# Sanoojan/REFace

Hardware: AMD Instinct MI355X
Metric: 512x512 50-step DDIM images/sec (higher is better)
Workload: dtype bf16; 1 GPU; BASELINE configs[1]: 512x512, 50 DDIM steps, CFG scale 3.5, batch 8 per GPU, bf16 UNet + fp32 VAE decode (bf16x3 MFMA operands), seeded random-init REFace weights; id=c1:512x512:S50:B8:bf16, batch_per_gpu=8, global_batch=8, ddim_steps=50, latent=64, parallelism=dp1 (pairs sharded, no collective in the step loop)

## Files before the change

### reface_amd/csrc/common.h

```cpp
#pragma once
#include <hip/hip_runtime.h>
#include <stdint.h>
#include <stdio.h>
#include <stdlib.h>
#include <string.h>

#include "../../include/reface_hip.h"

typedef __attribute__((ext_vector_type(8))) __bf16 bf16x8_t;
typedef __attribute__((ext_vector_type(16))) float f32x16_t;
typedef __attribute__((ext_vector_type(4))) float f32x4_t;
typedef __attribute__((ext_vector_type(4))) uint32_t u32x4_t;
typedef __attribute__((ext_vector_type(2))) uint32_t u32x2_t;

typedef uint16_t bf16_t;
typedef _Float16 f16_t;
typedef __attribute__((ext_vector_type(8))) _Float16 f16x8_t;
typedef uint8_t fp8_t;

namespace rf {

void set_error(const char* fmt, ...);


// ... 17 lines not shown
#define RF_RAISE_LDS(kernel, bytes, name)                                                                                                   \
    do {                                                                                                                                    \
        static unsigned long long done_ = 0ull;                                                                                             \
        int dev_ = 0;                                                                                                                       \
        (void)hipGetDevice(&dev_);                                                                                                          \
        const unsigned long long bit_ = 1ull << (dev_ & 63);                                                                                \
        if (!(done_ & bit_)) {                                                                                                              \
            const hipError_t e_ = hipFuncSetAttribute((const void*)(kernel), hipFuncAttributeMaxDynamicSharedMemorySize, (bytes));          \
            if (e_ != hipSuccess) {                                                                                                         \
                rf::set_error("%s: cannot raise the dynamic LDS limit to %d bytes on device %d: %s", name, (int)(bytes), dev_, hipGetErrorString(e_)); \
                return 2;                                                                                                                   \
            }                                                                                                                               \
            done_ |= bit_;                                                                                                                  \
        }                                                                                                                                   \
    } while (0)

__device__ __forceinline__ float as_f32(uint32_t x) { return __builtin_bit_cast(float, x); }
__device__ __forceinline__ uint32_t as_u32(float x) { return __builtin_bit_cast(uint32_t, x); }

typedef __attribute__((ext_vector_type(2))) __bf16 bf16x2_t;
__device__ __forceinline__ uint32_t pack_bf2(float lo, float hi) {
    const bf16x2_t v = {(__bf16)lo, (__bf16)hi};
    return __builtin_bit_cast(uint32_t, v);
}
__device__ __forceinline__ bf16_t f2bf(float f) { return __builtin_bit_cast(bf16_t, (__bf16)f); }
__device__ __forceinline__ float bf2f(bf16_t h) { return as_f32(((uint32_t)h) << 16); }

typedef __attribute__((ext_vector_type(2))) _Float16 f16x2_t;
__device__ __forceinline__ uint32_t pack_h2(float lo, float hi) {
    const f16x2_t v = {(_Float16)lo, (_Float16)hi};
    return __builtin_bit_cast(uint32_t, v);
}
template <typename T> __device__ __forceinline__ uint32_t pack2(float lo, float hi);
template <> __device__ __forceinline__ uint32_t pack2<bf16_t>(float lo, float hi) { return pack_bf2(lo, hi); }
template <> __device__ __forceinline__ uint32_t pack2<f16_t>(float lo, float hi) { return pack_h2(lo, hi); }
template <typename T> __device__ __forceinline__ float lo16(uint32_t w);
template <typename T> __device__ __forceinline__ float hi16(uint32_t w);
template <> __device__ __forceinline__ float lo16<bf16_t>(uint32_t w) { return as_f32(w << 16); }
template <> __device__ __forceinline__ float hi16<bf16_t>(uint32_t w) { return as_f32(w & 0xffff0000u); }
template <> __device__ __forceinline__ float lo16<f16_t>(uint32_t w) { return (float)__builtin_bit_cast(f16x2_t, w)[0]; }
template <> __device__ __forceinline__ float hi16<f16_t>(uint32_t w) { return (float)__builtin_bit_cast(f16x2_t, w)[1]; }
template <typename T> __device__ __forceinline__ float round16(float v);
template <> __device__ __forceinline__ float round16<bf16_t>(float v) { return bf2f(f2bf(v)); }
template <> __device__ __forceinline__ float round16<f16_t>(float v) { return (float)(_Float16)v; }
template <typename T> __device__ __forceinline__ constexpr uint16_t one16();
template <> __device__ __forceinline__ constexpr uint16_t one16<bf16_t>() { return 0x3f80; }
template <> __device__ __forceinline__ constexpr uint16_t one16<f16_t>() { return 0x3c00; }

__device__ __forceinline__ void split4_bf16(const float* f, u32x2_t& hi, u32x2_t& lo) {
    hi[0] = pack_bf2(f[0], f[1]);
    hi[1] = pack_bf2(f[2], f[3]);
    const float r0 = f[0] - as_f32(hi[0] << 16), r1 = f[1] - as_f32(hi[0] & 0xffff0000u);
    const float r2 = f[2] - as_f32(hi[1] << 16), r3 = f[3] - as_f32(hi[1] & 0xffff0000u);
    lo[0] = pack_bf2(r0, r1);
    lo[1] = pack_bf2(r2, r3);
}

__device__ __forceinline__ float quad_max(float v) {
    v = fmaxf(v, as_f32((uint32_t)__builtin_amdgcn_mov_dpp((int)as_u32(v), 0xB1, 0xF, 0xF, true)));
    v = fmaxf(v, as_f32((uint32_t)__builtin_amdgcn_mov_dpp((int)as_u32(v), 0x4E, 0xF, 0xF, true)));
    return v;
}
__device__ __forceinline__ int e8m0_for_amax(float amax) {
    const uint32_t b = as_u32(amax);
    int c = (int)((b >> 23) & 0xffu) - 8 + ((b & 0x7fffffu) > 0x600000u ? 1 : 0);
    return c < 0 ? 0 : (c > 253 ? 253 : c);
}
__device__ __forceinline__ u32x2_t quant8_fp8(const float* f, int code) {
    const float inv = as_f32((uint32_t)(254 - code) << 23);
    int lo = 0, hi = 0;
    lo = __builtin_amdgcn_cvt_pk_fp8_f32(f[0] * inv, f[1] * inv, lo, false);
    lo = __builtin_amdgcn_cvt_pk_fp8_f32(f[2] * inv, f[3] * inv, lo, true);
    hi = __builtin_amdgcn_cvt_pk_fp8_f32(f[4] * inv, f[5] * inv, hi, false);
    hi = __builtin_amdgcn_cvt_pk_fp8_f32(f[6] * inv, f[7] * inv, hi, true);
    return u32x2_t{(uint32_t)lo, (uint32_t)hi};
}
__device__ __forceinline__ void quant_block8(const float* f, fp8_t* qdst, fp8_t* sdst, bool quad_leader) {
    float m = 0.f;
#pragma unroll
    for (int e = 0; e < 8; ++e) m = fmaxf(m, fabsf(f[e]));
    const int code = e8m0_for_amax(quad_max(m));
    *(u32x2_t*)qdst = quant8_fp8(f, code);
    if (quad_leader) *sdst = (fp8_t)code;
}

template <typename T> struct elem;
template <> struct elem<float> {
    static constexpr int VEC = 4;
    __device__ static __forceinline__ float load(const float* p) { return *p; }
    __device__ static __forceinline__ void store(float* p, float v) { *p = v; }
};
template <> struct elem<fp8_t> {
    static constexpr int VEC = 16;
};
template <> struct elem<bf16_t> {
    static constexpr int VEC = 8;
    __device__ static __forceinline__ float load(const bf16_t* p) { return bf2f(*p); }
    __device__ static __forceinline__ void store(bf16_t* p, float v) { *p = f2bf(v); }
};

template <> struct elem<f16_t> {
    static constexpr int VEC = 8;
    __device__ static __forceinline__ float load(const f16_t* p) { return (float)*p; }
    __device__ static __forceinline__ void store(f16_t* p, float v) { *p = (f16_t)v; }
};

template <typename T> __device__ __forceinline__ void unpack16(const u32x4_t& v, float* f);
template <> __device__ __forceinline__ void unpack16<float>(const u32x4_t& v, float* f) {
#pragma unroll
    for (int i = 0; i < 4; ++i) f[i] = as_f32( v[i]);
}
template <> __device__ __forceinline__ void unpack16<bf16_t>(const u32x4_t& v, float* f) {
#pragma unroll
    for (int i = 0; i < 4; ++i) {
        f[2 * i] = as_f32( v[i] << 16);
        f[2 * i + 1] = as_f32( v[i] & 0xffff0000u);
    }
}
template <> __device__ __forceinline__ void unpack16<f16_t>(const u32x4_t& v, float* f) {
#pragma unroll
    for (int i = 0; i < 4; ++i) {
        const uint32_t w = v[i];
        f[2 * i] = lo16<f16_t>(w);
        f[2 * i + 1] = hi16<f16_t>(w);
    }
}
template <typename T> __device__ __forceinline__ u32x4_t pack16(const float* f);
template <> __device__ __forceinline__ u32x4_t pack16<float>(const float* f) {
    u32x4_t v;
#pragma unroll
    for (int i = 0; i < 4; ++i) v[i] = as_u32( f[i]);
    return v;
}
template <> __device__ __forceinline__ u32x4_t pack16<bf16_t>(const float* f) {
    u32x4_t v;
#pragma unroll
    for (int i = 0; i < 4; ++i) v[i] = pack_bf2(f[2 * i], f[2 * i + 1]);
    return v;
}

template <> __device__ __forceinline__ u32x4_t pack16<f16_t>(const float* f) {
    u32x4_t v;
#pragma unroll
    for (int i = 0; i < 4; ++i) v[i] = pack_h2(f[2 * i], f[2 * i + 1]);
    return v;
}

template <typename T> __device__ __forceinline__ void mma16(f32x16_t& acc, const u32x4_t& a, const u32x4_t& b);
template <> __device__ __forceinline__ void mma16<bf16_t>(f32x16_t& acc, const u32x4_t& a, const u32x4_t& b) {
    acc = __builtin_amdgcn_mfma_f32_32x32x16_bf16(__builtin_bit_cast(bf16x8_t, a), __builtin_bit_cast(bf16x8_t, b), acc, 0, 0, 0);
}
template <> __device__ __forceinline__ void mma16<f16_t>(f32x16_t& acc, const u32x4_t& a, const u32x4_t& b) {
    acc = __builtin_amdgcn_mfma_f32_32x32x16_f16(__builtin_bit_cast(f16x8_t, a), __builtin_bit_cast(f16x8_t, b), acc, 0, 0, 0);
}

__device__ __forceinline__ float silu_exact(float x) {
    const float e = __builtin_amdgcn_exp2f(x * -1.4426950408889634f);
    return x * __builtin_amdgcn_rcpf(1.0f + e);
}
__device__ __forceinline__ float erf_rational(float x) {
    x = fminf(fmaxf(x, -4.0f), 4.0f);
    const float x2 = x * x;
    float a = -2.72614225801306e-10f;
    a = fmaf(a, x2, 2.77068142495902e-08f);
    a = fmaf(a, x2, -2.10102402082508e-06f);
    a = fmaf(a, x2, -5.69250639462346e-05f);
    a = fmaf(a, x2, -7.34990630326855e-04f);
    a = fmaf(a, x2, -2.95459980854025e-03f);
    a = fmaf(a, x2, -1.60960333262415e-02f);
    float b = -1.45660718464996e-05f;
    b = fmaf(b, x2, -2.13374055278905e-04f);
    b = fmaf(b, x2, -1.68282697438203e-03f);
    b = fmaf(b, x2, -7.37332916720468e-03f);
    b = fmaf(b, x2, -1.42647390514189e-02f);
    return x * a * __builtin_amdgcn_rcpf(b);
}
__device__ __forceinline__ float gelu_erf(float x) { return 0.5f * x * (1.0f + erf_rational(x * 0.70710678118654752440f)); }
__device__ __forceinline__ float gelu_sigmoid5(float x) {
    const float xc = __builtin_fminf(__builtin_fmaxf(x, -7.0f), 7.0f);
    const float x2 = xc * xc;
    const float u = xc * __builtin_fmaf(__builtin_fmaf(-0.0010142630f, x2, 0.10677572f), x2, 2.3011212f);
    return x * __builtin_amdgcn_rcpf(1.0f + __builtin_amdgcn_exp2f(-u));
}
template <typename T> __device__ __forceinline__ float gelu_for(float x) {
    if constexpr (sizeof(T) == 2) return gelu_sigmoid5(x);
    else return gelu_erf(x);
}
__device__ __forceinline__ float quick_gelu(float x) { return x / (1.0f + expf(-1.702f * x)); }

__device__ __forceinline__ void halfwave_reduce_scatter32(float (&gx)[32], int lrow) {
#pragma unroll
    for (int st = 0; st < 5; ++st) {
        const int m = 16 >> st, n = 16 >> st;
        const unsigned up = (lrow & m) ? 0xffffffffu : 0u;
#pragma unroll
        for (int k = 0; k < n; ++k) {
            const unsigned a = __float_as_uint(gx[k]), b = __float_as_uint(gx[k + n]);
            const float send = __uint_as_float((a & up) | (b & ~up));
            const float keep = __uint_as_float((b & up) | (a & ~up));
            gx[k] = keep + __shfl_xor(send, m, 64);
        }
    }
}

__device__ __forceinline__ float wave_sum(float v) {
    v += as_f32((uint32_t)__builtin_amdgcn_mov_dpp((int)as_u32(v), 0xB1, 0xF, 0xF, true));
    v += as_f32((uint32_t)__builtin_amdgcn_mov_dpp((int)as_u32(v), 0x4E, 0xF, 0xF, true));
    v += as_f32((uint32_t)__builtin_amdgcn_mov_dpp((int)as_u32(v), 0x141, 0xF, 0xF, true));
    v += as_f32((uint32_t)__builtin_amdgcn_mov_dpp((int)as_u32(v), 0x140, 0xF, 0xF, true));
    {
        const auto r = __builtin_amdgcn_permlane16_swap(as_u32(v), as_u32(v), false, false);
        v = as_f32(r[0]) + as_f32(r[1]);
    }
    {
        const auto r = __builtin_amdgcn_permlane32_swap(as_u32(v), as_u32(v), false, false);
        v = as_f32(r[0]) + as_f32(r[1]);
    }
    return v;
}
__device__ __forceinline__ double wave_sum_d(double v) {
#pragma unroll
    for (int o = 32; o > 0; o >>= 1) v += __shfl_xor(v, o, 64);
    return v;
}
__device__ __forceinline__ float wave_max(float v) {
    v = fmaxf(v, as_f32((uint32_t)__builtin_amdgcn_mov_dpp((int)as_u32(v), 0xB1, 0xF, 0xF, true)));
    v = fmaxf(v, as_f32((uint32_t)__builtin_amdgcn_mov_dpp((int)as_u32(v), 0x4E, 0xF, 0xF, true)));
    v = fmaxf(v, as_f32((uint32_t)__builtin_amdgcn_mov_dpp((int)as_u32(v), 0x141, 0xF, 0xF, true)));
    v = fmaxf(v, as_f32((uint32_t)__builtin_amdgcn_mov_dpp((int)as_u32(v), 0x140, 0xF, 0xF, true)));
    {
        const auto r = __builtin_amdgcn_permlane16_swap(as_u32(v), as_u32(v), false, false);
        v = fmaxf(as_f32(r[0]), as_f32(r[1]));
    }
    {
        const auto r = __builtin_amdgcn_permlane32_swap(as_u32(v), as_u32(v), false, false);
        v = fmaxf(as_f32(r[0]), as_f32(r[1]));
    }
    return v;
}

}
```

### reface_amd/csrc/gemm.hip

```cpp
#include <cstdlib>
#include <type_traits>

#include "common.h"


namespace rf {
typedef float f32x2_t __attribute__((ext_vector_type(2)));

struct GemmParams {
    int M, N, K;
    const void* src0;
    const void* src1;
    int C0, Ctot, ld0, ld1;
    int Hin, Win, Hout, Wout, KH, KW, stride, pad_t, pad_l, ups;
    const void* W;
    int ldw;
    const float* bias;
    const float* rowvec;
    int rows_per_sample, ldv;
    const void* residual;
    int ldr, act;
    const float* act_vec;
    void* out;
    int ldo;
    float alpha;
    long long sA, sW, sO, sR;
    int tiles_m, tiles_n;
    unsigned a_bytes, w_bytes;
    int glds;
    int korder;
    int vec_ok;
    int splitk;
    float* ws;
    int pm, pn;
    int gn_rows;
    double* gn_part[2];
    int gn_cpg[2], gn_coff[2], gn_slot[2], gn_nch[2];
    int* plan;
    int epi2_ok;
    const float* wscale;
    void* oscale;
    int os_ld;
    const void* ascale;
    int as_ld;
    unsigned as_bytes;
    float* ln_out;
    int ln_out_parts;
    const float* ln_in;
    int ln_in_parts, ln_in_cols;
    float ln_eps;
    const float* ln_u;
    int x3;
    int lo_off;
    long long w_ps;
};

typedef __attribute__((ext_vector_type(2))) __bf16 bf16x2v_t;
__device__ __forceinline__ u32x4_t fp8x8_to_bf16x8(const u32x2_t& r, float scale) {
    u32x4_t o;
    o[0] = __builtin_bit_cast(uint32_t, __builtin_amdgcn_cvt_scalef32_pk_bf16_fp8(r[0], scale, false));
    o[1] = __builtin_bit_cast(uint32_t, __builtin_amdgcn_cvt_scalef32_pk_bf16_fp8(r[0], scale, true));
    o[2] = __builtin_bit_cast(uint32_t, __builtin_amdgcn_cvt_scalef32_pk_bf16_fp8(r[1], scale, false));
    o[3] = __builtin_bit_cast(uint32_t, __builtin_amdgcn_cvt_scalef32_pk_bf16_fp8(r[1], scale, true));
    return o;
}

template <typename T> struct MmaFrag;
template <> struct MmaFrag<bf16_t> {
    __device__ static __forceinline__ void mma(f32x16_t& acc, const u32x4_t& a, const u32x4_t& b) {
        acc = __builtin_amdgcn_mfma_f32_32x32x16_bf16(__builtin_bit_cast(bf16x8_t, a), __builtin_bit_cast(bf16x8_t, b), acc, 0, 0, 0);
    }
};
template <> struct MmaFrag<f16_t> {
    __device__ static __forceinline__ void mma(f32x16_t& acc, const u32x4_t& a, const u32x4_t& b) { mma16<f16_t>(acc, a, b); }
};
template <> struct MmaFrag<fp8_t> {
    __device__ static __forceinline__ void mma(f32x16_t&, const u32x4_t&, const u32x4_t&) {}
};
typedef int v8i_t __attribute__((ext_vector_type(8)));
__device__ __forceinline__ void mma_mx8(f32x16_t& acc, const u32x4_t& a0, const u32x4_t& a1, int sa, const u32x4_t& b0, const u32x4_t& b1, int sb) {
    const v8i_t a = {(int)a0[0], (int)a0[1], (int)a0[2], (int)a0[3], (int)a1[0], (int)a1[1], (int)a1[2], (int)a1[3]};
    const v8i_t b = {(int)b0[0], (int)b0[1], (int)b0[2], (int)b0[3], (int)b1[0], (int)b1[1], (int)b1[2], (int)b1[3]};
    asm volatile("s_nop 1\n\tv_mfma_scale_f32_32x32x64_f8f6f4 %0, %1, %2, %0, %3, %4 op_sel_hi:[0,0,0]" : "+v"(acc) : "v"(a), "v"(b), "v"(sa), "v"(sb));
}
template <> struct MmaFrag<float> {
    __device__ static __forceinline__ void mma(f32x16_t& acc, const u32x4_t& a, const u32x4_t& b) {
#pragma unroll
        for (int q = 0; q < 4; ++q)
            acc = __builtin_amdgcn_mfma_f32_32x32x2f32(as_f32( a[q]), as_f32( b[q]), acc, 0, 0, 0);
    }
};

__device__ __forceinline__ void lds_barrier() {
    asm volatile("s_waitcnt lgkmcnt(0)" ::: "memory");
    __builtin_amdgcn_s_barrier();
    asm volatile("" ::: "memory");
}

__device__ __forceinline__ int lds_off(int row, int slot) { return row * 128 + ((slot ^ ((row >> 1) & 7)) << 4); }

template <bool W8> __device__ __forceinline__ int w_stage(int t, int buf) { return W8 ? ((t >> 1) & 1) : buf; }
template <bool W8> __device__ __forceinline__ int w_soff(int t) { return (W8 ? (t >> 1) : t) * 128; }

template <typename TO> __device__ __forceinline__ void store_out(TO* p, float v);
template <> __device__ __forceinline__ void store_out<float>(float* p, float v) { *p = v; }
template <> __device__ __forceinline__ void store_out<bf16_t>(bf16_t* p, float v) { *p = f2bf(v); }
template <> __device__ __forceinline__ void store_out<f16_t>(f16_t* p, float v) { *p = (f16_t)v; }
template <typename TO> __device__ __forceinline__ float load_out(const TO* p);
template <> __device__ __forceinline__ float load_out<float>(const float* p) { return *p; }
template <> __device__ __forceinline__ float load_out<bf16_t>(const bf16_t* p) { return bf2f(*p); }
template <> __device__ __forceinline__ float load_out<f16_t>(const f16_t* p) { return (float)*p; }
template <typename X> struct is16 { static constexpr bool value = std::is_same<X, bf16_t>::value || std::is_same<X, f16_t>::value; };

template <typename T, typename TO, int WM, int WN, int TM, int TN, bool CONV, bool GLDS, int NST, int EPI = 0, bool W8 = false, int LNF = 0, bool HX = false>
__global__ __launch_bounds__(WM* WN * 64) void conv_gemm_kernel(const GemmParams p) {
    static_assert(LNF == 0 || (EPI == 1 && !CONV && !W8 && sizeof(T) == 2 && sizeof(TO) == 2), "LayerNorm folding: bf16 linear layers on the direct epilogue");
    static_assert(!HX || (CONV && GLDS && NST == 2 && sizeof(T) == 2 && !W8), "row-extended A tiles: bf16 3x3 convolutions on the two-stage direct-to-LDS loop");
    static_assert(EPI == 0 || GLDS, "the direct epilogue is built on the direct-to-LDS main loop");
    static_assert(!W8 || (GLDS && std::is_same<T, bf16_t>::value), "fp8 weights: bf16 activations on the direct-to-LDS main loop");
    constexpr bool A8 = std::is_same<T, fp8_t>::value;
    static_assert(!A8 || (GLDS && !W8 && NST == 2), "fp8 activations: direct-to-LDS main loop, two stages");
    constexpr int NT = WM * WN * 64;
    constexpr int BM = 32 * TM * WM;
    constexpr int BN = 32 * TN * WN;
    constexpr int VEC = elem<T>::VEC;
    constexpr int BK = 8 * VEC;
    constexpr int RPP = NT / 8;
    constexpr int AXR = HX ? ((BM * 5 / 4 + RPP - 1) / RPP) * RPP : BM;
    constexpr int AV = AXR / RPP;
    constexpr int BV = BN / RPP;
    static_assert(BM % RPP == 0 && BN % RPP == 0, "tile/threads mismatch");

    extern __shared__ __attribute__((aligned(16))) char smem[];
    char* const ldsA = smem;
    char* const ldsB = smem + NST * AXR * 128;
    char* const ldsS = smem + NST * (AXR + BN) * 128;

    const int tid = threadIdx.x;
    const int lane = tid & 63;
    const int wave = tid >> 6;
    const int wm = wave / WN, wn = wave % WN;

    int bid = blockIdx.x;
    {
        const int nwg = gridDim.x;
        const int q = nwg >> 3, r = nwg & 7, xcd = bid & 7, idx = bid >> 3;
        bid = (xcd < r ? xcd * (q + 1) : r * (q + 1) + (xcd - r) * q) + idx;
    }
    int tile_m, tile_n;
    {
        const int srow = p.pm * p.tiles_n;
        const int sr = bid / srow, rem = bid - sr * srow;
        const int h = min(p.pm, p.tiles_m - sr * p.pm);
        const int pw = h * p.pn;
        const int pc = rem / pw, r2 = rem - pc * pw;
        const int c = r2 / h;
        tile_m = sr * p.pm + (r2 - c * h);
        tile_n = pc * p.pn + c;
    }
    const int m0 = tile_m * BM, n0 = tile_n * BN;

    const long long zb = blockIdx.y;
    const T* src0 = (const T*)p.src0 + zb * p.sA;
    const T* src1 = (const T*)p.src1;
    const T* Wp = W8 ? (const T*)((const char*)p.W + zb * p.sW) : (const T*)p.W + zb * p.sW;
    if (!W8 && p.w_ps) Wp += (long long)(m0 / p.rows_per_sample) * p.w_ps;

    float colc = 0.f;
    if constexpr (EPI == 1) {
        if (tid < BN && n0 + tid < p.N && p.splitk == 1) {
            if (p.bias) colc = p.bias[n0 + tid];
            if (p.rowvec) colc += p.rowvec[(long long)(m0 / p.rows_per_sample) * p.ldv + n0 + tid];
        }
    }
    float colu = 0.f;
    if constexpr (LNF == 2) {
        if (tid < BN && n0 + tid < p.N) colu = p.ln_u[n0 + tid];
    }
    const int r0 = tid >> 3;
    const int slot = GLDS ? ((tid & 7) ^ ((r0 >> 1) & 7)) : (tid & 7);

    int a_pix[AV];
    int a_iy[AV], a_ix[AV];
#pragma unroll
    for (int i = 0; i < AV; ++i) {
        const int m = m0 + r0 + i * RPP;
        if (CONV) {
            const int hw = p.Hout * p.Wout;
            const int b = m / hw, rem = m - b * hw;
            const int oy = rem / p.Wout, ox = rem - oy * p.Wout;
            a_pix[i] = (m < p.M) ? b * p.Hin * p.Win : -1;
            a_iy[i] = oy * p.stride - p.pad_t;
            a_ix[i] = ox * p.stride - p.pad_l;
        } else {
            a_pix[i] = (m < p.M) ? m : -1;
            a_iy[i] = a_ix[i] = 0;
        }
    }
    int kvec = slot * VEC;
    int cv = kvec, ky = 0, kx = 0;
    if (CONV) {
        while (cv >= p.Ctot) {
            cv -= p.Ctot;
            if (++kx == p.KW) { kx = 0; ++ky; }
        }
    }
    const int Hv = p.ups ? p.Hin * 2 : p.Hin, Wv = p.ups ? p.Win * 2 : p.Win;

    auto advance_k = [&]() {
        kvec += BK;
        if (CONV) {
            if (p.korder) {
                if (++kx == p.KW) { kx = 0; if (++ky == p.KH) { ky = 0; cv += BK; } }
            } else {
                cv += BK;
                while (cv >= p.Ctot) {
                    cv -= p.Ctot;
                    if (++kx == p.KW) { kx = 0; ++ky; }
                }
            }
        }
    };

    u32x4_t ra[AV], rb[BV];

    auto load_tiles = [&]() {
        const bool kval = kvec < p.K;
#pragma unroll
        for (int i = 0; i < AV; ++i) {
            u32x4_t v = {0u, 0u, 0u, 0u};
            if (CONV) {
                int iy = a_iy[i] + ky, ix = a_ix[i] + kx;
                const bool ok = kval && a_pix[i] >= 0 && (unsigned)iy < (unsigned)Hv && (unsigned)ix < (unsigned)Wv;
                if (ok) {
                    if (p.ups) { iy >>= 1; ix >>= 1; }
                    const long long pix = (long long)a_pix[i] + iy * p.Win + ix;
                    const T* ptr = (cv < p.C0) ? src0 + pix * p.ld0 + cv : src1 + pix * p.ld1 + (cv - p.C0);
                    v = *(const u32x4_t*)ptr;
                }
            } else {
                if (kval && a_pix[i] >= 0) v = *(const u32x4_t*)(src0 + (long long)a_pix[i] * p.ld0 + kvec);
            }
            ra[i] = v;
        }
#pragma unroll
        for (int j = 0; j < BV; ++j) {
            const int n = n0 + r0 + j * RPP;
            u32x4_t v = {0u, 0u, 0u, 0u};
            if (kval && n < p.N) v = *(const u32x4_t*)(Wp + (long long)n * p.ldw + kvec);
            rb[j] = v;
        }
        advance_k();
    };
    auto store_tiles = [&](int buf) {
        char* a = ldsA + buf * BM * 128;
        char* b = ldsB + buf * BN * 128;
#pragma unroll
        for (int i = 0; i < AV; ++i) *(u32x4_t*)(a + lds_off(r0 + i * RPP, slot)) = ra[i];
#pragma unroll
        for (int j = 0; j < BV; ++j) *(u32x4_t*)(b + lds_off(r0 + j * RPP, slot)) = rb[j];
    };

    f32x16_t acc[TM][TN];
#pragma unroll
    for (int i = 0; i < TM; ++i)
#pragma unroll
        for (int j = 0; j < TN; ++j)
#pragma unroll
            for (int r = 0; r < 16; ++r) acc[i][j][r] = 0.0f;

    int nk = (p.K + BK - 1) / BK;
    int kb0_tiles = 0;
    if (p.splitk > 1) {
        int per = (nk + p.splitk - 1) / p.splitk;
        if (p.x3 || HX) per = (per + 2) / 3 * 3;
        const int kb0 = blockIdx.z * per;
        nk = max(0, min(nk, kb0 + per) - kb0);
        kb0_tiles = kb0;
        if (!GLDS)
            for (int i = 0; i < kb0; ++i) advance_k();
    }
    nk = __builtin_amdgcn_readfirstlane(nk);
    kb0_tiles = __builtin_amdgcn_readfirstlane(kb0_tiles);
    const int lrow = lane & 31, lhalf = lane >> 5;

    auto compute_tile = [&](int buf) {
        const char* a = ldsA + buf * BM * 128;
        const char* b = ldsB + buf * BN * 128;
#pragma unroll
        for (int kk = 0; kk < 4; ++kk) {
            const int s = kk * 2 + lhalf;
            u32x4_t fa[TM], fb[TN];
#pragma unroll
            for (int i = 0; i < TM; ++i) fa[i] = *(const u32x4_t*)(a + lds_off((wm * TM + i) * 32 + lrow, s));
#pragma unroll
            for (int j = 0; j < TN; ++j) fb[j] = *(const u32x4_t*)(b + lds_off((wn * TN + j) * 32 + lrow, s));
#pragma unroll
            for (int i = 0; i < TM; ++i)
#pragma unroll
                for (int j = 0; j < TN; ++j) MmaFrag<T>::mma(acc[i][j], fa[i], fb[j]);
        }
    };

    if constexpr (GLDS) {
        const __amdgpu_buffer_rsrc_t rsA = __builtin_amdgcn_make_buffer_rsrc((void*)src0, 0, p.a_bytes, 0x00020000);
        const __amdgpu_buffer_rsrc_t rsB = __builtin_amdgcn_make_buffer_rsrc((void*)Wp, 0, p.w_bytes, 0x00020000);
        constexpr int OOB = 0x7fffffff;
        constexpr int NP = AV + BV;
        static_assert(NP <= 20, "piece table too small");
        const int wave_u = __builtin_amdgcn_readfirstlane(wave);
        const int lane_k = slot * VEC * (int)sizeof(T);
        int offs[20];
        unsigned rowd[8];
        static_assert(AV <= 8, "row table too small");
        const __amdgpu_buffer_rsrc_t rsS = __builtin_amdgcn_make_buffer_rsrc((void*)(A8 ? p.ascale : (const void*)src0), 0, A8 ? p.as_bytes : 0u, 0x00020000);
        unsigned srowd = ~0u;
        int soffs = OOB;
        if constexpr (A8) {
            static_assert(BM <= NT, "one scale row per thread");
            const int srow = wave_u * 64 + lane, m = m0 + srow;
            const bool sv = srow < BM && m < p.M;
            if (CONV) {
                const int hw = p.Hout * p.Wout;
                const int b = m / hw, rem = m - b * hw;
                const int oy = rem / p.Wout, ox = rem - oy * p.Wout;
                srowd = sv ? ((unsigned)b << 20 | (unsigned)oy << 10 | (unsigned)ox) : ~0u;
            } else {
                soffs = sv ? m * p.as_ld : OOB;
            }
        }
#pragma unroll
        for (int j = 0; j < BV; ++j) {
            const int n = n0 + r0 + j * RPP;
            offs[AV + j] = n < p.N ? n * p.ldw * (W8 ? 1 : (int)sizeof(T)) + lane_k : OOB;
        }
        if (nk > 0) {
            char* const b0 = ldsB + w_stage<W8>(kb0_tiles, 0) * BN * 128 + wave_u * 1024;
            const int so0 = __builtin_amdgcn_readfirstlane(w_soff<W8>(kb0_tiles));
#pragma unroll
            for (int j = 0; j < BV; ++j)
                __builtin_amdgcn_raw_ptr_buffer_load_lds(rsB, (__attribute__((address_space(3))) void*)(b0 + j * (RPP * 128)), 16, offs[AV + j], so0, 0, 0);
        }
#pragma unroll
        for (int i = 0; i < AV; ++i) {
            const int m = m0 + r0 + i * RPP;
            if constexpr (HX) {
                const int j = r0 + i * RPP, we = p.Wout + 2;
                const int ir = j / we, xc = j - ir * we;
                const int R = m0 / p.Wout + ir;
                const int b = R / p.Hout, oy = R - b * p.Hout;
                rowd[i] = (ir < BM / p.Wout && R * p.Wout < p.M) ? ((unsigned)b << 20 | (unsigned)oy << 10 | (unsigned)xc) : ~0u;
            } else if (CONV) {
                const int hw = p.Hout * p.Wout;
                const int b = m / hw, rem = m - b * hw;
                const int oy = rem / p.Wout, ox = rem - oy * p.Wout;
                rowd[i] = m < p.M ? ((unsigned)b << 20 | (unsigned)oy << 10 | (unsigned)ox) : ~0u;
            } else {
                offs[i] = m < p.M ? m * p.ld0 * (int)sizeof(T) + lane_k : OOB;
            }
        }
        auto set_grp = [&](int dy) {
#pragma unroll
            for (int i = 0; i < AV; ++i) {
                const unsigned d = rowd[i];
                const int iy = (int)((d >> 10) & 1023u) + dy - 1, ix = (int)(d & 1023u) - 1;
                const bool ok = d != ~0u && (unsigned)iy < (unsigned)p.Hin && (unsigned)ix < (unsigned)p.Win;
                offs[i] = ok ? (((int)(d >> 20) * p.Hin + iy) * p.Win + ix) * p.ld0 * (int)sizeof(T) + lane_k : OOB;
            }
        };
        auto set_tap = [&](int ty, int tx) {
#pragma unroll
            for (int i = 0; i < AV; ++i) {
                const unsigned d = rowd[i];
                int iy = (int)((d >> 10) & 1023u) * p.stride - p.pad_t + ty;
                int ix = (int)(d & 1023u) * p.stride - p.pad_l + tx;
                const bool ok = d != ~0u && (unsigned)iy < (unsigned)Hv && (unsigned)ix < (unsigned)Wv;
                if (p.ups) { iy >>= 1; ix >>= 1; }
                offs[i] = ok ? (((int)(d >> 20) * p.Hin + iy) * p.Win + ix) * p.ld0 * (int)sizeof(T) + lane_k : OOB;
            }
            if constexpr (A8) {
                const unsigned d = srowd;
                int iy = (int)((d >> 10) & 1023u) * p.stride - p.pad_t + ty;
                int ix = (int)(d & 1023u) * p.stride - p.pad_l + tx;
                const bool ok = d != ~0u && (unsigned)iy < (unsigned)Hv && (unsigned)ix < (unsigned)Wv;
                if (p.ups) { iy >>= 1; ix >>= 1; }
                soffs = ok ? (((int)(d >> 20) * p.Hin + iy) * p.Win + ix) * p.as_ld : OOB;
            }
        };
        const int tpt = CONV ? p.Ctot / BK : 1;
        constexpr bool X3OK = sizeof(T) == 2 && sizeof(TO) == 4 && !W8 && NST == 2;
        const bool x3 = X3OK && p.x3;
        int it = kb0_tiles, ity = 0, itx = 0, ic = 0, ph = 0;
        int ia = x3 ? kb0_tiles / 3 : kb0_tiles;
        int hx_dx = 0, hx_ist = 0;
        if constexpr (HX) {
            const int grp = kb0_tiles / 3;
            ity = grp / tpt;
            ic = grp - ity * tpt;
            set_grp(ity);
        } else
        if (CONV) {
            const int ntap = p.KH * p.KW;
            const int tap = p.korder ? ia % ntap : ia / tpt;
            ic = p.korder ? ia / ntap : ia - tap * tpt;
            ity = tap / p.KW;
            itx = tap - ity * p.KW;
            set_tap(ity, itx);
        }
        auto next_tile = [&]() {
            ++it;
            if constexpr (HX) {
                if (++hx_dx == 3) {
                    hx_dx = 0;
                    hx_ist ^= 1;
                    if (++ic == tpt) { ic = 0; ++ity; set_grp(ity); }
                }
                return;
            }
            if (X3OK && x3) {
                if (++ph != 3) return;
                ph = 0;
            }
            ++ia;
            if (CONV) {
                if (p.korder) {
                    if (++itx == p.KW) { itx = 0; if (++ity == p.KH) { ity = 0; ++ic; } }
                    set_tap(ity, itx);
                } else if (++ic == tpt) {
                    ic = 0;
                    if (++itx == p.KW) { itx = 0; ++ity; }
                    set_tap(ity, itx);
                }
            }
        };
        auto issue_pieces = [&](int buf, int q0, int q1) {
            char* a = ldsA + (HX ? hx_ist : buf) * AXR * 128 + wave_u * 1024;
            char* b = ldsB + w_stage<W8>(it, buf) * BN * 128 + wave_u * 1024;
            const int soA = __builtin_amdgcn_readfirstlane((CONV ? ic : ia) * 128 + ((X3OK && ph == 2) ? p.lo_off : 0));
            const int soB = __builtin_amdgcn_readfirstlane(w_soff<W8>(it));
            if (W8 && (it & 1) && q1 > AV) q1 = AV;
#pragma unroll
            for (int q = 0; q < NP; ++q) {
                if (q >= q0 && q < q1) {
                    if (q < AV) {
                        if (!(HX && hx_dx != 0))
                            __builtin_amdgcn_raw_ptr_buffer_load_lds(rsA, (__attribute__((address_space(3))) void*)(a + q * (RPP * 128)), 16, offs[q], soA, 0, 0);
                    } else
                        __builtin_amdgcn_raw_ptr_buffer_load_lds(rsB, (__attribute__((address_space(3))) void*)(b + (q - AV) * (RPP * 128)), 16, offs[q], soB, 0, 0);
                }
            }
            if (A8 && q0 == 0) {
                char* const sdst = ldsS + buf * 2048 + wave_u * 256;
                const int soS = __builtin_amdgcn_readfirstlane((CONV ? ic : ia) * 4);
                __builtin_amdgcn_raw_ptr_buffer_load_lds(rsS, (__attribute__((address_space(3))) void*)sdst, 4, soffs, soS, 0, 0);
            }
        };
        if constexpr (A8) {
            using std::integral_constant;
            constexpr int JS8 = TN > 2 ? 2 : 1;
            u32x4_t fa8[2][TM][2], fb8[TN][2];
            int sa8[2][TM], wsc[TN];
            const int lrow_ = lane & 31, lhalf_ = lane >> 5;
            const int frag_sw8 = (lrow_ >> 1) & 7;
            const int brow8 = EPI == 1 ? (16 * ((lrow_ >> 2) & 1) + 4 * (lrow_ >> 3) + (lrow_ & 3)) : lrow_;
            const int frag_swb8 = (brow8 >> 1) & 7;
            int fk8[2], fkb8[2], ssh[2];
#pragma unroll
            for (int kk = 0; kk < 2; ++kk) {
                fk8[kk] = ((4 * kk + lhalf_) ^ frag_sw8) << 4;
                fkb8[kk] = ((4 * kk + lhalf_) ^ frag_swb8) << 4;
                ssh[kk] = (2 * kk + lhalf_) * 8;
            }
#pragma unroll
            for (int j = 0; j < TN; ++j) {
                const int n = n0 + (wn * TN + j) * 32 + brow8;
                wsc[j] = n < p.N ? (int)((as_u32(p.wscale[n]) >> 23) & 0xffu) : 127;
            }
            const char* curA = ldsA + (wm * TM) * 4096 + lrow_ * 128;
            const char* curB = ldsB + (wn * TN) * 4096 + brow8 * 128;
            const char* curS = ldsS + ((wm * TM) * 32 + lrow_) * 4;
            const char* othA = curA + BM * 128;
            const char* othB = curB + BN * 128;
            const char* othS = curS + 2048;
            auto ld_a = [&](int buf, const char* bA, const char* bS, int kk) {
#pragma unroll
                for (int i = 0; i < TM; ++i) {
                    fa8[buf][i][0] = *(const u32x4_t*)(bA + i * 4096 + fk8[kk]);
                    fa8[buf][i][1] = *(const u32x4_t*)(bA + i * 4096 + (fk8[kk] ^ 32));
                    sa8[buf][i] = (int)((*(const uint32_t*)(bS + i * 128) >> ssh[kk]) & 0xffu);
                }
            };
            auto ld_b = [&](int j, const char* bB, int kk) {
                fb8[j][0] = *(const u32x4_t*)(bB + j * 4096 + fkb8[kk]);
                fb8[j][1] = *(const u32x4_t*)(bB + j * 4096 + (fkb8[kk] ^ 32));
            };
            auto mma_col = [&](int buf, int j) {
#pragma unroll
                for (int i = 0; i < TM; ++i) {
                    if constexpr (EPI == 1) mma_mx8(acc[i][j], fb8[j][0], fb8[j][1], wsc[j], fa8[buf][i][0], fa8[buf][i][1], sa8[buf][i]);
                    else mma_mx8(acc[i][j], fa8[buf][i][0], fa8[buf][i][1], sa8[buf][i], fb8[j][0], fb8[j][1], wsc[j]);
                }
            };
            auto phase8 = [&](auto KK, int stage, bool more) {
                constexpr int kk = decltype(KK)::value;
                constexpr int cur = kk, nx = kk ^ 1, nkk = kk ^ 1;
                const char* const nA = kk == 0 ? curA : othA;
                const char* const nB = kk == 0 ? curB : othB;
                const char* const nS = kk == 0 ? curS : othS;
#pragma unroll
                for (int j = 0; j < JS8; ++j) mma_col(cur, j);
                if (kk == 1) {
                    asm volatile("s_waitcnt vmcnt(0) lgkmcnt(0)" ::: "memory");
                    __builtin_amdgcn_s_barrier();
                }
                ld_a(nx, nA, nS, nkk);
#pragma unroll
                for (int j = 0; j < JS8; ++j) ld_b(j, nB, nkk);
                __builtin_amdgcn_sched_barrier(0);
#pragma unroll
                for (int j = JS8; j < TN; ++j) {
                    mma_col(cur, j);
                    ld_b(j, nB, nkk);
                    if (kk == 1) {
                        constexpr int COLS = TN - JS8, PPC = (NP + COLS - 1) / COLS;
                        if (more) issue_pieces(stage, (j - JS8) * PPC, (j - JS8 + 1) * PPC < NP ? (j - JS8 + 1) * PPC : NP);
                    }
                    __builtin_amdgcn_sched_barrier(0);
                }
                __builtin_amdgcn_sched_barrier(0);
            };
            if (nk > 0) {
                issue_pieces(0, 0, AV);
                if (nk > 1) {
                    next_tile();
                    issue_pieces(1, 0, NP);
                    if (nk > 2) next_tile();
                    asm volatile("s_waitcnt vmcnt(%0)" ::"n"(NP + 1) : "memory");
                } else {
                    asm volatile("s_waitcnt vmcnt(0)" ::: "memory");
                }
                __builtin_amdgcn_s_barrier();
                ld_a(0, curA, curS, 0);
#pragma unroll
                for (int j = 0; j < TN; ++j) ld_b(j, curB, 0);
            }
            for (int kt = 0; kt < nk; ++kt) {
                const int stage = kt & 1;
                const bool more = kt + 2 < nk;
                phase8(integral_constant<int, 0>{}, stage, more);
                phase8(integral_constant<int, 1>{}, stage, more);
                if (kt + 3 < nk) next_tile();
                const char* t = curA; curA = othA; othA = t;
                t = curB; curB = othB; othB = t;
                t = curS; curS = othS; othS = t;
            }
            asm volatile("s_nop 15\n\ts_nop 15" ::: "memory");
            __syncthreads();
        } else {
        constexpr bool ROT = TM * TN > 8;
        constexpr int JS = ROT ? 2 : 0;
        u32x4_t fa[2][TM], fb[W8 ? 1 : 2][W8 ? 1 : TN];
        u32x2_t fbr[W8 ? 2 : 1][W8 ? TN : 1];
        float ws[W8 ? TN : 1];
        const int frag_sw = (lrow >> 1) & 7;
        const int brow = EPI == 1 ? (16 * ((lrow >> 2) & 1) + 4 * (lrow >> 3) + (lrow & 3)) : lrow;
        const int frag_swb = (brow >> 1) & 7;
        int fk[4], fkb[4];
#pragma unroll
        for (int kk = 0; kk < 4; ++kk) {
            fk[kk] = ((kk * 2 + lhalf) ^ frag_sw) << 4;
            fkb[kk] = W8 ? (((kk ^ frag_swb) << 4) + lhalf * 8) : (((kk * 2 + lhalf) ^ frag_swb) << 4);
        }
        if constexpr (W8) {
#pragma unroll
            for (int j = 0; j < TN; ++j) {
                const int n = n0 + (wn * TN + j) * 32 + brow;
                ws[j] = n < p.N ? p.wscale[n] : 1.0f;
            }
        }
        const char* curA = ldsA + (wm * TM) * 4096 + lrow * 128;
        int erow[TM];
        const char* hcb[TM];
        const char* hnb[TM];
        int hcs[TM], hns[TM], m_dx = 0, m_st = 0;
        const int ks_[4] = {(0 + lhalf) << 4, (2 + lhalf) << 4, (4 + lhalf) << 4, (6 + lhalf) << 4};
        auto hx_set = [&](const char** hb, int* hs, int st, int dx) {
#pragma unroll
            for (int i = 0; i < TM; ++i) {
                const int e = erow[i] + dx;
                hb[i] = ldsA + st * (AXR * 128) + e * 128;
                hs[i] = ((e >> 1) & 7) << 4;
            }
        };
        if constexpr (HX) {
#pragma unroll
            for (int i = 0; i < TM; ++i) {
                const int pm = (wm * TM + i) * 32 + lrow, ir = pm / p.Wout;
                erow[i] = ir * (p.Wout + 2) + (pm - ir * p.Wout);
            }
            hx_set(hcb, hcs, 0, 0);
            hx_set(hnb, hns, 0, 1);
        }
        const char* const wbase = ldsB + (wn * TN) * 4096 + brow * 128;
        const char* curB = wbase + w_stage<W8>(kb0_tiles, 0) * BN * 128;
        const char* othA = curA + BM * 128;
        const char* othB = wbase + w_stage<W8>(kb0_tiles + 1, 1) * BN * 128;
        int curPar = W8 ? (kb0_tiles & 1) * 64 : 0, othPar = W8 ? ((kb0_tiles + 1) & 1) * 64 : 0;
        int t_abs = kb0_tiles;
        auto load_b = [&](int set, int j, const char* ptr) {
            if constexpr (W8) fbr[set][j] = *(const u32x2_t*)ptr;
            else fb[set][j] = *(const u32x4_t*)ptr;
        };
        auto bfrag = [&](int set, int j) -> u32x4_t {
            if constexpr (W8) return fp8x8_to_bf16x8(fbr[set][j], ws[j]);
            else return fb[set][j];
        };
        auto phase = [&](auto KK, int stage, bool more, bool deep) {
            constexpr int kk = decltype(KK)::value;
            constexpr int cur = kk & 1, nx = cur ^ 1;
            constexpr int fbc = ROT ? 0 : cur, fbn = ROT ? 0 : nx;
            constexpr int nkk = (kk + 1) & 3;
            const char* const nA = (kk < 3 ? curA : othA) + fk[nkk];
            const char* const nB = (kk < 3 ? curB : othB) + (fkb[nkk] ^ (kk < 3 ? curPar : othPar));
#pragma unroll
            for (int j = 0; j < JS; ++j) {
                const u32x4_t bj = bfrag(fbc, j);
#pragma unroll
                for (int i = 0; i < TM; ++i) {
                    if constexpr (EPI == 1) MmaFrag<T>::mma(acc[i][j], bj, fa[cur][i]);
                    else MmaFrag<T>::mma(acc[i][j], fa[cur][i], bj);
                }
            }
            if (kk == 3) {
                if (NST > 2 && deep) asm volatile("s_waitcnt vmcnt(%0) lgkmcnt(0)" ::"n"((NST - 2) * NP) : "memory");
                else asm volatile("s_waitcnt vmcnt(0) lgkmcnt(0)" ::: "memory");
                __builtin_amdgcn_s_barrier();
            }
#pragma unroll
            for (int i = 0; i < TM; ++i) {
                if constexpr (HX) fa[nx][i] = *(const u32x4_t*)((kk < 3 ? hcb[i] : hnb[i]) + (ks_[nkk] ^ (kk < 3 ? hcs[i] : hns[i])));
                else fa[nx][i] = *(const u32x4_t*)(nA + i * 4096);
            }
#pragma unroll
            for (int j = 0; j < (ROT ? JS : TN); ++j) load_b(fbn, j, nB + j * 4096);
            __builtin_amdgcn_sched_barrier(0);
#pragma unroll
            for (int j = JS; j < TN; ++j) {
                const u32x4_t bj = bfrag(fbc, j);
#pragma unroll
                for (int i = 0; i < TM; ++i) {
                    if constexpr (EPI == 1) MmaFrag<T>::mma(acc[i][j], bj, fa[cur][i]);
                    else MmaFrag<T>::mma(acc[i][j], fa[cur][i], bj);
                }
                if (ROT) load_b(0, j, nB + j * 4096);
                if (kk == 3) {
                    constexpr int COLS = TN - JS, PPC = (NP + COLS - 1) / COLS;
                    if (more) issue_pieces(stage, (j - JS) * PPC, (j - JS + 1) * PPC < NP ? (j - JS + 1) * PPC : NP);
                }
                if (ROT || kk == 3) __builtin_amdgcn_sched_barrier(0);
            }
            __builtin_amdgcn_sched_barrier(0);
        };
        using std::integral_constant;
        if (nk > 0) {
            issue_pieces(0, 0, AV);
            if constexpr (NST > 2) {
                static_assert(!W8, "the deep ring is for bf16 / fp32 weights");
#pragma unroll
                for (int s = 1; s < NST; ++s)
                    if (s < nk) {
                        next_tile();
                        issue_pieces(s, 0, NP);
                    }
                if (nk > NST) next_tile();
                if (nk >= NST) asm volatile("s_waitcnt vmcnt(%0)" ::"n"((NST - 1) * NP) : "memory");
                else asm volatile("s_waitcnt vmcnt(0)" ::: "memory");
            } else if (nk > 1) {
                next_tile();
                issue_pieces(1, 0, NP);
                if (nk > 2) next_tile();
                if constexpr (W8) asm volatile("s_waitcnt vmcnt(0)" ::: "memory");
                else asm volatile("s_waitcnt vmcnt(%0)" ::"n"(HX ? BV : NP) : "memory");
            } else {
                asm volatile("s_waitcnt vmcnt(0)" ::: "memory");
            }
            __builtin_amdgcn_s_barrier();
#pragma unroll
            for (int i = 0; i < TM; ++i) {
                if constexpr (HX) fa[0][i] = *(const u32x4_t*)(hcb[i] + (ks_[0] ^ hcs[i]));
                else fa[0][i] = *(const u32x4_t*)(curA + i * 4096 + fk[0]);
            }
#pragma unroll
            for (int j = 0; j < TN; ++j) load_b(0, j, curB + j * 4096 + (fkb[0] ^ curPar));
        }
        if constexpr (NST > 2) {
            const char* const baseA = curA;
            int sc = 0, so = 1;
            for (int kt = 0; kt < nk; ++kt) {
                const bool more = kt + NST < nk, deep = kt + NST - 1 < nk;
                phase(integral_constant<int, 0>{}, sc, more, deep);
                phase(integral_constant<int, 1>{}, sc, more, deep);
                phase(integral_constant<int, 2>{}, sc, more, deep);
                phase(integral_constant<int, 3>{}, sc, more, deep);
                if (kt + NST + 1 < nk) next_tile();
                sc = so;
                so = so + 1 == NST ? 0 : so + 1;
                curA = othA; othA = baseA + so * (BM * 128);
                curB = othB; othB = wbase + so * (BN * 128);
            }
        } else {
// ... 1210 lines not shown
```

Measured before the change: 9.799 images/s.

## Use 16x16x32 MFMA tiles for bf16/f16 GEMM main loop

Adds a main-loop path for 16-bit operand GEMMs and convolutions that splits each 32x32 warp tile into four 16x16 MFMA tiles using the 16x16x32 bf16/f16 instructions. Fragment addressing in LDS is reworked, and after the loop the results are remapped into the existing 32x32 accumulator layout with permlane16 swaps so the epilogues stay unchanged. The aim is higher MFMA throughput or better LDS access and latency hiding for bf16 layers. In exchange it adds more accumulator registers, more fragment loads and extra permute work per tile.

```diff
diff --git a/reface_amd/csrc/common.h b/reface_amd/csrc/common.h
--- a/reface_amd/csrc/common.h
+++ b/reface_amd/csrc/common.h
@@ -193,6 +193,13 @@
 }
 template <> __device__ __forceinline__ void mma16<f16_t>(f32x16_t& acc, const u32x4_t& a, const u32x4_t& b) {
     acc = __builtin_amdgcn_mfma_f32_32x32x16_f16(__builtin_bit_cast(f16x8_t, a), __builtin_bit_cast(f16x8_t, b), acc, 0, 0, 0);
+}
+template <typename T> __device__ __forceinline__ void mma16x16(f32x4_t& acc, const u32x4_t& a, const u32x4_t& b);
+template <> __device__ __forceinline__ void mma16x16<bf16_t>(f32x4_t& acc, const u32x4_t& a, const u32x4_t& b) {
+    acc = __builtin_amdgcn_mfma_f32_16x16x32_bf16(__builtin_bit_cast(bf16x8_t, a), __builtin_bit_cast(bf16x8_t, b), acc, 0, 0, 0);
+}
+template <> __device__ __forceinline__ void mma16x16<f16_t>(f32x4_t& acc, const u32x4_t& a, const u32x4_t& b) {
+    acc = __builtin_amdgcn_mfma_f32_16x16x32_f16(__builtin_bit_cast(f16x8_t, a), __builtin_bit_cast(f16x8_t, b), acc, 0, 0, 0);
 }
 
 __device__ __forceinline__ float silu_exact(float x) {
diff --git a/reface_amd/csrc/gemm.hip b/reface_amd/csrc/gemm.hip
--- a/reface_amd/csrc/gemm.hip
+++ b/reface_amd/csrc/gemm.hip
@@ -99,6 +99,23 @@
 
 __device__ __forceinline__ int lds_off(int row, int slot) { return row * 128 + ((slot ^ ((row >> 1) & 7)) << 4); }
 
+struct Frag16 {
+    __device__ static __forceinline__ int slot(int kk, int g) { return ((8 - 2 * g) & 7) | kk; }
+    __device__ static __forceinline__ int col_row(int h, int c) { return 16 * h + c; }
+    template <bool EPI1> __device__ static __forceinline__ int row_row(int h, int c) {
+        return EPI1 ? 8 * (c >> 2) + 4 * h + (c & 3) : 16 * ((c >> 2) & 1) + 8 * h + 4 * (c >> 3) + (c & 3);
+    }
+    __device__ static __forceinline__ void to_acc32(f32x16_t& acc, const f32x4_t& x0, const f32x4_t& x1, int h) {
+#pragma unroll
+        for (int r = 0; r < 4; ++r) {
+            const float a = x0[r], b = x1[r];
+            const auto s = __builtin_amdgcn_permlane16_swap(as_u32(a), as_u32(b), false, false);
+            acc[4 * h + r] = as_f32(s[0]);
+            acc[8 + 4 * h + r] = as_f32(s[1]);
+        }
+    }
+};
+
 template <bool W8> __device__ __forceinline__ int w_stage(int t, int buf) { return W8 ? ((t >> 1) & 1) : buf; }
 template <bool W8> __device__ __forceinline__ int w_soff(int t) { return (W8 ? (t >> 1) : t) * 128; }
 
@@ -389,6 +406,7 @@
         };
         const int tpt = CONV ? p.Ctot / BK : 1;
         constexpr bool X3OK = sizeof(T) == 2 && sizeof(TO) == 4 && !W8 && NST == 2;
+        constexpr bool MF16 = sizeof(T) == 2;
         const bool x3 = X3OK && p.x3;
         int it = kb0_tiles, ity = 0, itx = 0, ic = 0, ph = 0;
         int ia = x3 ? kb0_tiles / 3 : kb0_tiles;
@@ -556,6 +574,225 @@
             }
             asm volatile("s_nop 15\n\ts_nop 15" ::: "memory");
             __syncthreads();
+        } else if constexpr (MF16) {
+            constexpr int MI = 2 * TM, MJ = 2 * TN;
+            constexpr bool ROT = TM * TN > 8;
+            static_assert(!ROT || MJ >= 6, "the rotating loop needs middle columns");
+            constexpr int FS = ROT ? 1 : 2;
+            f32x4_t c16[MI][MJ];
+#pragma unroll
+            for (int i = 0; i < MI; ++i)
+#pragma unroll
+                for (int j = 0; j < MJ; ++j) c16[i][j] = f32x4_t{0.f, 0.f, 0.f, 0.f};
+            u32x4_t fa[FS][MI], fb[W8 ? 1 : FS][W8 ? 1 : MJ];
+            u32x2_t fbr[W8 ? FS : 1][W8 ? MJ : 1];
+            float ws[W8 ? MJ : 1];
+            const int fc = lane & 15, fg = lane >> 4;
+            int afk[2], wfk[2], arow[2];
+#pragma unroll
+            for (int h = 0; h < 2; ++h) {
+                arow[h] = EPI == 1 ? Frag16::col_row(h, fc) : Frag16::row_row<false>(h, fc);
+                afk[h] = lds_off(arow[h], Frag16::slot(0, fg));
+                const int wr = EPI == 1 ? Frag16::row_row<true>(h, fc) : Frag16::col_row(h, fc);
+                wfk[h] = W8 ? lds_off(wr, Frag16::slot(0, fg) >> 1) : lds_off(wr, Frag16::slot(0, fg));
+                if constexpr (W8) {
+#pragma unroll
+                    for (int j = h; j < MJ; j += 2) {
+                        const int n = n0 + (wn * TN + (j >> 1)) * 32 + wr;
+                        ws[j] = n < p.N ? p.wscale[n] : 1.0f;
+                    }
+                }
+            }
+            const int sl16 = Frag16::slot(0, fg) << 4;
+            const int wm_u = wave_u / WN, wn_u = wave_u % WN;
+            const char* curA = ldsA + (wm_u * TM) * 4096;
+            const char* othA = curA + BM * 128;
+            const char* const wbase = ldsB + (wn_u * TN) * 4096;
+            const char* curB = wbase + w_stage<W8>(kb0_tiles, 0) * BN * 128;
+            const char* othB = wbase + w_stage<W8>(kb0_tiles + 1, 1) * BN * 128;
+            int curPar = W8 ? (kb0_tiles & 1) * 64 : 0, othPar = W8 ? ((kb0_tiles + 1) & 1) * 64 : 0;
+            int t_abs = kb0_tiles;
+            int erow[HX ? MI : 1];
+            const char* hcb[HX ? MI : 1];
+            const char* hnb[HX ? MI : 1];
+            int hcs[HX ? MI : 1], hns[HX ? MI : 1], m_dx = 0, m_st = 0;
+            auto hx_set = [&](const char** hb, int* hs, int st, int dx) {
+#pragma unroll
+                for (int i = 0; i < MI; ++i) {
+                    const int e = erow[i] + dx;
+                    hb[i] = ldsA + st * (AXR * 128) + e * 128;
+                    hs[i] = ((e >> 1) & 7) << 4;
+                }
+            };
+            if constexpr (HX) {
+#pragma unroll
+                for (int i = 0; i < MI; ++i) {
+                    const int pm = (wm * TM + (i >> 1)) * 32 + arow[i & 1], ir = pm / p.Wout;
+                    erow[i] = ir * (p.Wout + 2) + (pm - ir * p.Wout);
+                }
+                hx_set(hcb, hcs, 0, 0);
+                hx_set(hnb, hns, 0, 1);
+            }
+            auto ld_a = [&](int set, int i, int kk, const char* base, bool nxt) {
+                if constexpr (HX) fa[set][i] = *(const u32x4_t*)((nxt ? hnb[i] : hcb[i]) + ((sl16 ^ (kk << 4)) ^ (nxt ? hns[i] : hcs[i])));
+                else fa[set][i] = *(const u32x4_t*)(base + (i >> 1) * 4096 + (afk[i & 1] ^ (kk << 4)));
+            };
+            auto ld_b = [&](int set, int j, int kk, const char* base, int par) {
+                if constexpr (W8) fbr[set][j] = *(const u32x2_t*)(base + (j >> 1) * 4096 + ((wfk[j & 1] ^ par) + 8 * kk));
+                else fb[set][j] = *(const u32x4_t*)(base + (j >> 1) * 4096 + (wfk[j & 1] ^ (kk << 4)));
+            };
+            auto bfrag = [&](int set, int j) -> u32x4_t {
+                if constexpr (W8) return fp8x8_to_bf16x8(fbr[set][j], ws[j]);
+                else return fb[set][j];
+            };
+            auto mma_b = [&](int set, int i, int j, const u32x4_t& b) {
+                if constexpr (EPI == 1) mma16x16<T>(c16[i][j], b, fa[set][i]);
+                else mma16x16<T>(c16[i][j], fa[set][i], b);
+            };
+            auto tile_barrier = [&](bool deep) {
+                if (NST > 2 && deep) asm volatile("s_waitcnt vmcnt(%0) lgkmcnt(0)" ::"n"((NST - 2) * NP) : "memory");
+                else asm volatile("s_waitcnt vmcnt(0) lgkmcnt(0)" ::: "memory");
+                __builtin_amdgcn_s_barrier();
+            };
+            auto step = [&](auto KK, int stage, bool more, bool deep) {
+                constexpr int kk = decltype(KK)::value, nkk = kk ^ 1;
+                const char* const nA = kk == 0 ? curA : othA;
+                const char* const nB = kk == 0 ? curB : othB;
+                const int nPar = kk == 0 ? curPar : othPar;
+                if constexpr (ROT) {
+                    {
+                        const u32x4_t b0 = bfrag(0, 0), b1 = bfrag(0, 1);
+#pragma unroll
+                        for (int i = 0; i < MI; ++i) { mma_b(0, i, 0, b0); mma_b(0, i, 1, b1); }
+                    }
+                    __builtin_amdgcn_sched_barrier(0);
+                    if (kk == 1) tile_barrier(deep);
+#pragma unroll
+                    for (int j = 2; j < MJ - 2; ++j) {
+                        const u32x4_t bj = bfrag(0, j);
+#pragma unroll
+                        for (int i = 0; i < MI; ++i) {
+                            mma_b(0, i, j, bj);
+                            if (i == 0 && j < 4) ld_b(0, j - 2, nkk, nB, nPar);
+                        }
+                        ld_b(0, j, nkk, nB, nPar);
+                        if (kk == 1) {
+                            constexpr int COLS = MJ - 4, PPC = (NP + COLS - 1) / COLS;
+                            if (more) issue_pieces(stage, (j - 2) * PPC, (j - 1) * PPC < NP ? (j - 1) * PPC : NP);
+                        }
+                        __builtin_amdgcn_sched_barrier(0);
+                    }
+                    {
+                        const u32x4_t b0 = bfrag(0, MJ - 2), b1 = bfrag(0, MJ - 1);
+#pragma unroll
+                        for (int i = 0; i < MI; ++i) {
+                            mma_b(0, i, MJ - 2, b0);
+                            mma_b(0, i, MJ - 1, b1);
+                            ld_a(0, i, nkk, nA, kk == 1);
+                            __builtin_amdgcn_sched_barrier(0);
+                        }
+                    }
+                    ld_b(0, MJ - 2, nkk, nB, nPar);
+                    ld_b(0, MJ - 1, nkk, nB, nPar);
+                } else {
+                    constexpr int cur = kk, nx = kk ^ 1;
+                    if (kk == 1) tile_barrier(deep);
+#pragma unroll
+                    for (int j = 0; j < MJ; ++j) {
+                        const u32x4_t bj = bfrag(cur, j);
+#pragma unroll
+                        for (int i = 0; i < MI; ++i) {
+                            mma_b(cur, i, j, bj);
+                            const int q = j * MI + i;
+                            if (q < MI) ld_a(nx, q, nkk, nA, kk == 1);
+                            else if (q < MI + MJ) ld_b(nx, q - MI, nkk, nB, nPar);
+                        }
+                        if (kk == 1) {
+                            constexpr int PPC = (NP + MJ - 1) / MJ;
+                            if (more) issue_pieces(stage, j * PPC < NP ? j * PPC : NP, (j + 1) * PPC < NP ? (j + 1) * PPC : NP);
+                        }
+                        __builtin_amdgcn_sched_barrier(0);
+                    }
+                }
+                __builtin_amdgcn_sched_barrier(0);
+            };
+            using std::integral_constant;
+            if (nk > 0) {
+                issue_pieces(0, 0, AV);
+                if constexpr (NST > 2) {
+                    static_assert(!W8, "the deep ring is for bf16 / fp32 weights");
+#pragma unroll
+                    for (int s = 1; s < NST; ++s)
+                        if (s < nk) {
+                            next_tile();
+                            issue_pieces(s, 0, NP);
+                        }
+                    if (nk > NST) next_tile();
+                    if (nk >= NST) asm volatile("s_waitcnt vmcnt(%0)" ::"n"((NST - 1) * NP) : "memory");
+                    else asm volatile("s_waitcnt vmcnt(0)" ::: "memory");
+                } else if (nk > 1) {
+                    next_tile();
+                    issue_pieces(1, 0, NP);
+                    if (nk > 2) next_tile();
+                    if constexpr (W8) asm volatile("s_waitcnt vmcnt(0)" ::: "memory");
+                    else asm volatile("s_waitcnt vmcnt(%0)" ::"n"(HX ? BV : NP) : "memory");
+                } else {
+                    asm volatile("s_waitcnt vmcnt(0)" ::: "memory");
+                }
+                __builtin_amdgcn_s_barrier();
+#pragma unroll
+                for (int i = 0; i < MI; ++i) ld_a(0, i, 0, curA, false);
+#pragma unroll
+                for (int j = 0; j < MJ; ++j) ld_b(0, j, 0, curB, curPar);
+            }
+            if constexpr (NST > 2) {
+                const char* const baseA = curA;
+                const char* const baseB = wbase;
+                int sc = 0, so = 1;
+                for (int kt = 0; kt < nk; ++kt) {
+                    const bool more = kt + NST < nk, deep = kt + NST - 1 < nk;
+                    step(integral_constant<int, 0>{}, sc, more, deep);
+                    step(integral_constant<int, 1>{}, sc, more, deep);
+                    if (kt + NST + 1 < nk) next_tile();
+                    sc = so;
+                    so = so + 1 == NST ? 0 : so + 1;
+                    curA = othA; othA = baseA + so * (BM * 128);
+                    curB = othB; othB = baseB + so * (BN * 128);
+                }
+            } else {
+                for (int kt = 0; kt < nk; ++kt) {
+                    const int stage = kt & 1;
+                    const bool more = kt + 2 < nk;
+                    step(integral_constant<int, 0>{}, stage, more, false);
+                    step(integral_constant<int, 1>{}, stage, more, false);
+                    if (kt + 3 < nk) next_tile();
+                    const char* t = curA; curA = othA; othA = t;
+                    if constexpr (W8) {
+                        ++t_abs;
+                        curB = othB; curPar = othPar;
+                        othB = wbase + (((t_abs + 1) >> 1) & 1) * BN * 128;
+                        othPar = ((t_abs + 1) & 1) * 64;
+                    } else {
+                        t = curB; curB = othB; othB = t;
+                    }
+                    if constexpr (HX) {
+                        if (++m_dx == 3) { m_dx = 0; m_st ^= 1; }
+#pragma unroll
+                        for (int i = 0; i < MI; ++i) { hcb[i] = hnb[i]; hcs[i] = hns[i]; }
+                        hx_set(hnb, hns, m_dx == 2 ? (m_st ^ 1) : m_st, m_dx == 2 ? 0 : m_dx + 1);
+                    }
+                }
+            }
+            __syncthreads();
+#pragma unroll
+            for (int i = 0; i < TM; ++i)
+#pragma unroll
+                for (int j = 0; j < TN; ++j)
+#pragma unroll
+                    for (int h = 0; h < 2; ++h) {
+                        if constexpr (EPI == 1) Frag16::to_acc32(acc[i][j], c16[2 * i][2 * j + h], c16[2 * i + 1][2 * j + h], h);
+                        else Frag16::to_acc32(acc[i][j], c16[2 * i + h][2 * j], c16[2 * i + h][2 * j + 1], h);
+                    }
         } else {
         constexpr bool ROT = TM * TN > 8;
         constexpr int JS = ROT ? 2 : 0;
```

Result: slower. 9.685 images/s, median of 2 (-1.2%).
